# nmichlo/mtg-vision

Hardware: AMD Instinct MI355X
Metric: cards/sec end-to-end (detect+embed+top-1 over 100k bank), 640x640 (higher is better)
Workload: dtype f32 (products as 3 x f16 MFMA on hi/lo-split operands, f32 accumulate)

## Files before the change

### mtg-vision_amd/csrc/gemm_sp.hip

```cpp
#include "gemm_sp.h"

#include <stdlib.h>
#include <map>
#include <mutex>
#include <vector>

#include "gemm_sp_kernel.h"

namespace mtgv {

__global__ __launch_bounds__(256) void sp8_pack_rows_kernel(const float* __restrict__ in, sp_h8* __restrict__ out,
                                                           float* __restrict__ wscale, long rows, int K) {
  const int lane = threadIdx.x & 63;
  const long row = (long)blockIdx.x * 4 + (threadIdx.x >> 6);
  if (row >= rows) return;
  const float* x = in + row * K;
  float mx = 0.f;
  for (int k = lane; k < K; k += 64) mx = fmaxf(mx, fabsf(x[k]));
#pragma unroll
  for (int m = 32; m > 0; m >>= 1) mx = fmaxf(mx, __shfl_xor(mx, m));
  int e = 0;
  if (mx > 0.f && mx < INFINITY) {
    int ex;
    (void)frexpf(mx, &ex);
// ... 114 lines not shown
void gemm_sp_launch_cfg2(const SpDev& g, int amode, hipStream_t s);
void gemm_sp_launch_cfg3(const SpDev& g, int amode, hipStream_t s);
void gemm_sp_launch_cfg4(const SpDev& g, int amode, hipStream_t s);
void gemm_sp_launch_cfg5(const SpDev& g, int amode, hipStream_t s);
void gemm_sp_launch_cfg6(const SpDev& g, int amode, hipStream_t s);

namespace {
struct SpCfg {
  int wm, wn, tm, tn;
  double eff;
  int ks = 2;
  int bm() const { return 32 * tm * wm; }
  int bn() const { return 32 * tn * wn; }
  int rb() const { return 64 * ks; }
  int kps() const { return 16 * ks; }
};
const SpCfg kCfg[] = {
    {2, 2, 2, 2, 0.93},
    {2, 2, 2, 3, 1.00},
    {4, 1, 1, 3, 0.88},
    {4, 1, 1, 2, 0.80},
    {4, 1, 1, 1, 0.62},
    {4, 2, 1, 3, 0.00},
    {4, 1, 1, 1, 0.00, 1},
};
constexpr int kNumCfg = sizeof(kCfg) / sizeof(kCfg[0]);
}

bool window_conv_on() {
  static const bool on = [] { const char* e = getenv("MTGV_SP_WINDOW"); return e == nullptr || atoi(e) != 0; }();
  return on;
}

static size_t window_bytes(const SpCfg& k, int Wd) {
  const int rpp = 1024 / k.rb();
  return (size_t)((k.bm() + 2 * Wd + 2 + rpp - 1) / rpp * rpp) * k.rb();
}

bool window_conv_fits(const GemmArgs& a, const SpPlan& pl) {
  const SpCfg& k = kCfg[pl.cfg];
  if (!(window_conv_on() && a.KH == 3 && a.KW == 3 && a.stride == 1 && a.pad == 1 && a.stride_w <= 0 && a.Cin % k.kps() == 0 &&
        a.OH == a.H && a.OW == a.Wd))
    return false;
  return window_bytes(k, a.Wd) + (size_t)2 * k.bn() * k.rb() <= 80 * 1024;
}

bool gemm_sp_active() { return gemm_precision() == GEMM_PREC_F16X3; }

bool gemm_sp_takes_sp8(const float* W, int M, int N, int K, int lda, int c_off) {
  if (!gemm_sp_active()) return false;
  if (K % 8 != 0 || N % 4 != 0 || lda % 8 != 0 || c_off % 8 != 0 || M <= 0) return false;
  return sp8_lookup(W, K, nullptr, nullptr);
}

static int chain_cfg(const GemmArgs& a) {
  if (a.W2 == nullptr || a.Out2 == nullptr || !is_conv(a)) return -1;
  if (!(gemm_sp_active() && a.a_fmt == 1 && a.act == ACT_SILU && a.res == nullptr && a.grn_part == nullptr && a.topk == 0 && a.batch == 1 &&
        a.os == 1 && a.os_nq == 0 && a.OH2 == a.OH && a.OW2 == a.OW && a.a_scale == nullptr && a.ln_w == nullptr))
    return -1;
  if (!(a.N == 32 || a.N == 64 || a.N == 96) || a.N2 <= 0 || a.N2 % 32 != 0 || a.N2 > a.N) return -1;
  if (a.K % 8 != 0 || a.c_total % 8 != 0 || a.c_off % 8 != 0 || a.ldo2 % 4 != 0 || a.o_off2 % 4 != 0 || ((uintptr_t)a.Out2 & 15) != 0) return -1;
  if (a.out_fmt2 == 1 && (a.ldo2 % 8 != 0 || a.o_off2 % 8 != 0)) return -1;
  if (a.stride_w > 0 || a.Cin % 8 != 0) return -1;
  if (!sp8_lookup(a.W, a.K, nullptr, nullptr) || !sp8_lookup(a.W2, a.N, nullptr, nullptr)) return -1;
  return a.N == 32 ? 4 : (a.N == 64 ? 3 : 2);
}
bool gemm_sp_chain_ok(const GemmArgs& a) { return chain_cfg(a) >= 0; }

SpPlan gemm_sp_plan(const GemmArgs& a) {
  SpPlan pl;
  if (a.W2 != nullptr) {
    const int c = chain_cfg(a);
    MTGV_CHECK(c >= 0, ERR_INVALID, "gemm: this launch cannot chain its second layer (M=%d N=%d K=%d N2=%d): ask gemm_sp_chain_ok first", a.M,
               a.N, a.K, a.N2);
    const SpCfg& k = kCfg[c];
    pl.cfg = c, pl.bm = k.bm(), pl.bn = k.bn(), pl.unit_rows = 32 * k.tm;
    pl.tiles_m = ceil_div(a.M, k.bm()), pl.tiles_n = 1;
    return pl;
// ... 61 lines not shown
  if (best == 1 && !conv && sp8_in && a.grn_part != nullptr && a.topk == 0 && a.K >= 256 && a.M >= 12288) best = 5;
  const SpCfg& k = kCfg[best];
  pl.cfg = best;
  pl.bm = k.bm(), pl.bn = k.bn();
  pl.unit_rows = 32 * k.tm;
  pl.tiles_m = ceil_div(a.M, k.bm());
  pl.tiles_n = ceil_div(a.N, k.bn());
  return pl;
}

namespace {
struct StampRec { int M, N, K, cfg, amode, act, tiles; long* buf; };
std::vector<StampRec> g_stamps;
bool stamps_on() {
  static const bool on = [] { const char* e = getenv("MTGV_SP_STAMPS"); return e != nullptr && atoi(e) != 0; }();
  return on;
}
}

bool gemm_sp_topk_layout(const GemmArgs& a, int* slots, int* cols) {
  const SpPlan pl = gemm_sp_plan(a);
  if (pl.cfg < 0) return false;
  const SpCfg& k = kCfg[pl.cfg];
  *slots = pl.tiles_n * k.wn;
  *cols = 32 * k.tn;
  return true;
}

double gemm_sp_fill_bytes(const GemmArgs& a, const SpPlan& pl) {
  const SpCfg& k = kCfg[pl.cfg];
  const double tiles = (double)pl.tiles_m * pl.tiles_n;
  const double b_tile = (double)k.bn() * a.K * 4.0;
  double a_tile = (double)k.bm() * a.K * 4.0;
  if (a.a_fmt == 1 && is_conv(a) && window_conv_fits(a, pl)) a_tile = (double)window_bytes(k, a.Wd) * (a.Cin / k.kps());
  if (a.a_scale != nullptr) a_tile += (double)(a.K / 32) * 1024.0;
  return tiles * (a_tile + b_tile);
}

void gemm_sp_stamps_dump(const char* path) {
  if (g_stamps.empty()) return;
  HIP_OK(hipDeviceSynchronize());
  FILE* f = fopen(path, "wb");
  MTGV_CHECK(f != nullptr, ERR_RUNTIME, "cannot open %s", path);
  std::vector<long> host;
  for (const StampRec& r : g_stamps) {
    const int hdr[8] = {r.M, r.N, r.K, r.cfg, r.amode, r.act, r.tiles, 0};
    fwrite(hdr, sizeof(int), 8, f);
    host.resize((size_t)r.tiles * 8);
    HIP_OK(hipMemcpy(host.data(), r.buf, host.size() * sizeof(long), hipMemcpyDeviceToHost));
    fwrite(host.data(), sizeof(long), host.size(), f);
    HIP_OK(hipFree(r.buf));
  }
  fclose(f);
  g_stamps.clear();
}

int gemm_sp_topk_hi16_range_cols() { return 32 * kCfg[1].tn; }
int gemm_sp_topk_hi16_slots(int N) { return ceil_div(N, kCfg[1].bn()) * kCfg[1].wn; }

void gemm_sp_topk_hi16_launch(const void* q_hi, const void* bank_hi, const float* wscale, int b, int N, int K, int kp, float* cand_s,
                              int* cand_i, int* slots, hipStream_t s) {
  const SpCfg& k1 = kCfg[1];
  MTGV_CHECK(b >= 128 && N >= k1.bn() && K % 64 == 0 && kp >= 1 && kp <= 32 * k1.tn, ERR_INVALID, "topk_hi16: b=%d N=%d K=%d kp=%d", b, N, K, kp);
  MTGV_CHECK(((uintptr_t)q_hi & 15) == 0 && ((uintptr_t)bank_hi & 15) == 0, ERR_INVALID, "topk_hi16: operands must be 16-byte aligned");
  SpDev g;
  g.A = reinterpret_cast<const char*>(q_hi);
  g.a_rowb = (long)K * 2;
// ... 36 lines not shown
  g.d_hw = make_fastdiv((uint32_t)g.hw);
  g.a_scale = a.a_scale;
  g.a_mul = a.a_fmt == 1 ? 1.0f : a.a_mul;
  g.a_unmul = a.a_fmt == 1 ? 1.0f : a.a_unmul;
  g.zero = sp_zero_page();
  {
    const double lim = 4294967296.0 - 65536.0;
    g.off32 = ((double)a.M * g.a_rowb + (double)g.a_offb < lim && (double)a.N * a.K * 4.0 < lim) ? 1 : 0;
  }
  g.tiles_m = pl.tiles_m, g.tiles_n = pl.tiles_n;
  g.cand_s = a.cand_s, g.cand_i = a.cand_i, g.topk = a.topk;
  g.act = a.act;
  g.H = a.H, g.Wd = a.Wd, g.Cin = a.Cin, g.KW = a.KW, g.stride = a.stride, g.pad = a.pad, g.OH = a.OH, g.OW = a.OW;
  g.d_ohw = make_fastdiv((uint32_t)(a.OH * a.OW));
  g.d_ow = make_fastdiv((uint32_t)a.OW);
  g.d_cin = make_fastdiv((uint32_t)(a.Cin > 0 ? a.Cin : 1));
  g.d_kw = make_fastdiv((uint32_t)a.KW);
  g.remap = is_remap(a);
  g.os = a.os, g.oy = a.oy, g.ox = a.ox, g.OH2 = a.OH2, g.OW2 = a.OW2;
  if (a.W2 != nullptr) {
    const char* w28 = nullptr;
    const float* w2s = nullptr;
    MTGV_CHECK(sp8_lookup(a.W2, a.N, &w28, &w2s), ERR_RUNTIME, "gemm_sp: second-layer weights lost their SP8 copy");
    g.W2 = w28, g.wscale2 = w2s, g.bias2 = a.bias2, g.Out2 = a.Out2, g.ldo2 = a.ldo2, g.o_off2 = a.o_off2, g.out_fmt2 = a.out_fmt2;
    g.act2 = a.act2, g.N2 = a.N2;
  }
  g.nq = a.os_nq;
  g.d_nq = make_fastdiv((uint32_t)(a.os_nq > 0 ? a.os_nq : 1)), g.d_os = make_fastdiv((uint32_t)(a.os > 0 ? a.os : 1));
  if (a.os_nq > 0)
    MTGV_CHECK(g.remap && a.os_nq % 8 == 0 && a.N == a.os * a.os * a.os_nq && a.oy == 0 && a.ox == 0 && a.res == nullptr &&
                   a.grn_part == nullptr,
               ERR_INVALID, "gemm_sp: os_nq=%d does not describe a %dx%d scatter of N=%d columns", a.os_nq, a.os, a.os, a.N);
  int amode = a.a_fmt == 1 ? (is_conv(a) ? 2 : 0) : 1;
  if (amode == 2 && window_conv_fits(a, pl)) amode = 5;
  if (amode == 1 && g.a_mul == 1.0f && ((uintptr_t)g.A & 15) == 0) {
    if (g.a_scale == nullptr) amode = 4;
    else if (((uintptr_t)g.a_scale & 15) == 0 && (kCfg[pl.cfg].bm() - 1) / g.hw + 2 <= 8) amode = 3;
  }
  if (stamps_on() && gemm_profile_enabled()) {
    const int tiles = pl.tiles_m * pl.tiles_n;
    long* buf = nullptr;
    HIP_OK(hipMalloc(&buf, (size_t)tiles * 8 * sizeof(long)));
    HIP_OK(hipMemsetAsync(buf, 0, (size_t)tiles * 8 * sizeof(long), s));
    g.stamps = buf;
    g_stamps.push_back({a.M, a.N, a.K, pl.cfg, amode, a.act, tiles, buf});
  }
  switch (pl.cfg) {
    case 0: gemm_sp_launch_cfg0(g, amode, s); break;
    case 1: gemm_sp_launch_cfg1(g, amode, s); break;
    case 2: gemm_sp_launch_cfg2(g, amode, s); break;
    case 3: gemm_sp_launch_cfg3(g, amode, s); break;
    case 4: gemm_sp_launch_cfg4(g, amode, s); break;
    case 5: gemm_sp_launch_cfg5(g, amode, s); break;
    case 6: gemm_sp_launch_cfg6(g, amode, s); break;
    default: MTGV_CHECK(false, ERR_INVALID, "gemm_sp: bad cfg %d", pl.cfg);
  }
  HIP_OK(hipGetLastError());
}

}
```

### mtg-vision_amd/csrc/gemm_sp_inst.h

```cpp
#pragma once
#include "gemm_sp_kernel.h"

namespace mtgv {

namespace {
#ifndef SP_KS_VALUE
#define SP_KS_VALUE 2
#endif
constexpr int SP_KS = SP_KS_VALUE;
#ifndef SP_NST
#define SP_NST 2
#endif

template <int AMODE, int ACT, int EPI, int NST = SP_NST>
void sp_launch_nst(const SpDev& g, hipStream_t s) {
  constexpr int BM = 32 * SP_TM * SP_WM, BN = 32 * SP_TN * SP_WN;
  constexpr size_t ring = (size_t)NST * ((AMODE == 5 ? BN : BM + BN) * 64 * SP_KS + (AMODE == 3 ? 1024 : 0));
  size_t lds = ring;
  constexpr size_t chain_lds = (size_t)SP_WM * SP_WN * 4096 * (1 + SP_TN) + (size_t)SP_TN * 96 * 128;
  if (AMODE == 5) {
    constexpr int RB = 64 * SP_KS, RPP = 1024 / RB;
    const size_t win = (size_t)((BM + 2 * g.Wd + 2 + RPP - 1) / RPP * RPP) * RB;
    const size_t stage = (size_t)SP_WM * SP_WN * 32 * 128 * SP_TN;
    lds = win + ring > stage ? win + ring : stage;
  }
  if (EPI == 32 && lds < chain_lds) lds = chain_lds;
  static bool attr_done_dev[MTGV_MAX_DEVICES] = {};
  bool& attr_done = attr_done_dev[current_device()];
  auto kern = gemm_sp_kernel<SP_WM, SP_WN, SP_TM, SP_TN, SP_KS, NST, AMODE, ACT, EPI>;
  if (!attr_done) {
    HIP_OK(hipFuncSetAttribute((const void*)kern, hipFuncAttributeMaxDynamicSharedMemorySize, (AMODE == 5 || EPI == 32) ? 160 * 1024 : (int)lds));
    attr_done = true;
  }
  hipLaunchKernelGGL(kern, dim3((unsigned)(g.tiles_m * g.tiles_n)), dim3(64 * SP_WM * SP_WN), lds, s, g);
}

template <int AMODE, int ACT, int EPI>
void sp_launch_one(const SpDev& g, hipStream_t s) {
  if constexpr (AMODE == 5 && SP_NST == 2) {
    constexpr int BM = 32 * SP_TM * SP_WM, BN = 32 * SP_TN * SP_WN, RB = 64 * SP_KS, RPP = 1024 / RB;
    const size_t win = (size_t)((BM + 2 * g.Wd + 2 + RPP - 1) / RPP * RPP) * RB;
    if ((long)g.tiles_m * g.tiles_n <= 512 && win + (size_t)4 * BN * RB <= 80 * 1024) {
      sp_launch_nst<AMODE, ACT, EPI, 4>(g, s);
      return;
    }
  }
  sp_launch_nst<AMODE, ACT, EPI, SP_NST>(g, s);
}

int sp_epi_of(const SpDev& g) {
  if (g.W2 != nullptr) return 32;
  if (g.remap || g.N % 4 != 0) return -1;
  return (g.out_fmt == 1 ? 1 : 0) | (g.res != nullptr ? (g.res_fmt == 1 ? 4 : 2) : 0) | (g.grn_part != nullptr ? 8 : 0);
}

template <int AMODE, int ACT>
void sp_pick(const SpDev& g, int epi, hipStream_t s) {
  MTGV_CHECK(epi != 32, ERR_RUNTIME, "gemm_sp: no chained-1x1 instance for A mode %d in configuration %d", AMODE, SP_CFG_ID);
  sp_launch_one<AMODE, ACT, -1>(g, s);
}
template <int AMODE, int ACT, int E0, int... ES>
void sp_pick(const SpDev& g, int epi, hipStream_t s) {
  if (epi == E0) sp_launch_one<AMODE, ACT, E0>(g, s);
  else sp_pick<AMODE, ACT, ES...>(g, epi, s);
}
}

#define SP_CAT2(a, b) a##b
#define SP_CAT(a, b) SP_CAT2(a, b)

void SP_CAT(gemm_sp_launch_cfg, SP_CFG_ID)(const SpDev& g, int amode, hipStream_t s) {
  if (g.topk > 0) {
#if SP_CFG_ID == 1
    MTGV_CHECK((amode == 4 || amode == 6) && g.act == ACT_NONE, ERR_INVALID, "gemm_sp: top-k needs aligned f32 queries");
// ... 73 lines not shown
```

### mtg-vision_amd/csrc/gemm_sp_kernel.h

```cpp
#pragma once
#include <type_traits>

#include "act.h"
#include "gemm_f32.h"
#include "sp8.h"

namespace mtgv {

typedef float spf16 __attribute__((ext_vector_type(16)));

__device__ __forceinline__ spf16 sp_mfma(sp_h8 b, sp_h8 a, spf16 c) {
  return __builtin_amdgcn_mfma_f32_32x32x16_f16(b, a, c, 0, 0, 0);
}

struct SpDev {
  float* cand_s = nullptr;
  int* cand_i = nullptr;
  int topk = 0;
  long* stamps = nullptr;
  const char* A = nullptr;
  long a_rowb = 0;
  long a_offb = 0;
  const char* W = nullptr;
  const float* wscale = nullptr;
  const float* bias = nullptr;
  const void* res = nullptr;
  long ldr = 0;
  int res_fmt = 0;
  float* Out = nullptr;
  long ldo = 0;
  int o_off = 0;
  int out_fmt = 0;
  int M = 0, N = 0, K = 0;
  float* grn_part = nullptr;
  int hw = 1, segmax = 0;
  FastDiv d_hw;
  const float* a_scale = nullptr;
  float a_mul = 1.0f, a_unmul = 1.0f;
  const char* zero = nullptr;
  int off32 = 0;
  int tiles_m = 0, tiles_n = 0;
  int act = 0;
  int H = 1, Wd = 1, Cin = 0, KW = 1, stride = 1, pad = 0, OH = 1, OW = 1;
  FastDiv d_ohw, d_ow, d_cin, d_kw;
  int remap = 0, os = 1, oy = 0, ox = 0, OH2 = 1, OW2 = 1;
  int nq = 0;
  FastDiv d_nq, d_os;
  const char* W2 = nullptr;
  const float* wscale2 = nullptr;
  const float* bias2 = nullptr;
  float* Out2 = nullptr;
  long ldo2 = 0;
  int o_off2 = 0, out_fmt2 = 0, act2 = 0, N2 = 0;
};

typedef const __attribute__((address_space(1))) void* sp_gptr;
typedef __attribute__((address_space(3))) void* sp_lptr;

template <int WM, int WN, int TM, int TN, int KS, int NST, int AMODE, int ACT, int EPI>
__global__ __launch_bounds__(64 * WM * WN, (WM * WN == 8 ? 4 : 2)) void gemm_sp_kernel(const SpDev g) {
#pragma clang fp contract(off)
  constexpr int NW = WM * WN, NT = 64 * NW, BM = 32 * TM * WM, BN = 32 * TN * WN;
  constexpr bool GEN = EPI < 0;
  static_assert(TM <= 2, "the epilogue names its slabs");
  static_assert(NST >= 2 && NST <= 4 && (AMODE != 1 || NST == 2), "ring depth; the register A path is two-deep");
  constexpr int RB = 64 * KS, RPP = 1024 / RB, SPR = RB / 16;
  constexpr bool AWIN = AMODE == 5;
  constexpr bool ADMA = AMODE != 1 && !AWIN;
  constexpr bool AF32 = AMODE == 3 || AMODE == 4;
  constexpr bool HI16 = AMODE == 6;
  constexpr int EB = HI16 ? 2 : 4;
  static_assert(!HI16 || (KS == 2 && EPI == 16), "fp16 rows: 128-byte stage rows, top-k epilogue");
  constexpr int SA = AWIN ? 0 : BM * RB, SB = BN * RB, SSC = AMODE == 3 ? 1024 : 0, STG = SA + SB + SSC;
  static_assert(AMODE != 3 || KS == 2, "the scale image is one DMA piece: 8 images x 32 k");
  constexpr int PA = ADMA ? BM / RPP : 0, PB = BN / RPP, NP = PA + PB;
  constexpr int PPW = (NP + NW - 1) / NW;
  constexpr int CPS = BM * 2 * KS;
  constexpr int CPT = AMODE == 1 ? CPS / NT : 1;
  static_assert(AMODE != 1 || CPS % NT == 0, "A chunks must divide over the threads");
  extern __shared__ __attribute__((aligned(1024))) char smem[];

  const int tid = threadIdx.x, lane = tid & 63;
  const int wave = __builtin_amdgcn_readfirstlane(tid >> 6);
  const int wm = wave / WN, wn = wave % WN;
  const int r = lane & 31, h = lane >> 5;

  const long st0 = g.stamps != nullptr ? (long)__builtin_amdgcn_s_memtime() : 0;
  const long rt0 = g.stamps != nullptr ? (long)__builtin_amdgcn_s_memrealtime() : 0;
  long st1 = 0;
  int L;
  {
    const int nwg = gridDim.x, b = blockIdx.x;
    const int q = nwg >> 3, rr = nwg & 7, x = b & 7;
    L = (x < rr ? x * (q + 1) : rr * (q + 1) + (x - rr) * q) + (b >> 3);
  }
  const int tile_n = L % g.tiles_n, tile_m = L / g.tiles_n;
  const int m0 = tile_m * BM, n0 = tile_n * BN;
  const long wrowb = (long)g.K * EB;
  const int kchunks = g.K >> 3;
  constexpr int KPS = 16 * KS * (4 / EB);
  const int nk = (g.K + KPS - 1) / KPS;
  const bool ktail = (g.K % KPS) != 0;

  const char* src[PPW];
  bool tailz[PPW];
  int cslot[PPW], cih0[PPW], ciw0[PPW];
  const char* csrc[PPW];
  const bool conv_fast = AMODE == 2 && g.Cin % (16 * KS) == 0;
  uint32_t off32[PPW];
  const bool sfast = g.off32 != 0 && !ktail;
#pragma unroll
  for (int u = 0; u < PPW; ++u) {
    const int p = wave + NW * u;
    const bool isA = p < PA;
    const int pp = isA ? p : p - PA;
    const int row = pp * RPP + lane / SPR;
    const int sw = KS == 2 ? (row >> 1) & 7 : (row >> 2) & 3;
    const int slot = (lane % SPR) ^ sw;
    cslot[u] = slot, cih0[u] = 0, ciw0[u] = 0, csrc[u] = nullptr;
    {
      const int mm = m0 + row < g.M ? m0 + row : g.M - 1, nn = n0 + row < g.N ? n0 + row : g.N - 1;
      off32[u] = isA ? (uint32_t)mm * (uint32_t)g.a_rowb + (uint32_t)(slot * 16) : (uint32_t)nn * (uint32_t)wrowb + (uint32_t)(slot * 16);
    }
    if (isA) {
      int m = m0 + row;
      m = m < g.M ? m : g.M - 1;
      if constexpr (AMODE == 2) {
        const uint32_t img = fdiv((uint32_t)m, g.d_ohw);
        const uint32_t rem = (uint32_t)m - img * (uint32_t)(g.OH * g.OW);
        const uint32_t oh = fdiv(rem, g.d_ow);
        const uint32_t ow = rem - oh * (uint32_t)g.OW;
        cih0[u] = (int)oh * g.stride - g.pad;
        ciw0[u] = (int)ow * g.stride - g.pad;
        csrc[u] = g.A + (((long)img * g.H + cih0[u]) * g.Wd + ciw0[u]) * g.a_rowb + g.a_offb + slot * 16;
        src[u] = g.A + (long)img * g.H * g.Wd * g.a_rowb + g.a_offb + (slot & 1) * 16;
      } else {
        src[u] = g.A + (long)m * g.a_rowb + g.a_offb + slot * 16;
      }
    } else {
      int n = n0 + row;
      n = n < g.N ? n : g.N - 1;
      src[u] = g.W + (long)n * wrowb + slot * 16;
    }
    tailz[u] = ktail && ((nk - 1) * 2 * KS + (slot >> 1)) >= kchunks;
  }
  const int img0 = AMODE == 3 ? (int)fdiv((uint32_t)m0, g.d_hw) : 0;
  const char* sc_src = nullptr;
  bool sc_tailz = false;
  if constexpr (AMODE == 3) {
    const int img_last = (int)fdiv((uint32_t)(g.M - 1), g.d_hw);
    const int im = img0 + (lane >> 3) < img_last ? img0 + (lane >> 3) : img_last;
    sc_src = reinterpret_cast<const char*>(g.a_scale + (long)im * g.K) + (lane & 7) * 16;
    sc_tailz = ktail && ((nk - 1) * 2 * KS + ((lane & 7) >> 1)) >= kchunks;
  }
  const int win_px = AWIN ? ((BM + 2 * g.Wd + 2 + RPP - 1) / RPP * RPP) : 0;
  char* const ring = smem + (AWIN ? win_px * RB : 0);
  auto issue_piece = [&](int u, int t, int buf) {
    const int p = wave + NW * u;
    const char* s;
    if (AMODE == 2 && p < PA && conv_fast) {
      const uint32_t k0 = (uint32_t)t * (16u * KS);
      const uint32_t tap = fdiv(k0, g.d_cin);
      const uint32_t kh = fdiv(tap, g.d_kw);
      const uint32_t kw = tap - kh * (uint32_t)g.KW;
      const long tap_off = ((long)kh * g.Wd + kw) * g.a_rowb + (long)(k0 - tap * (uint32_t)g.Cin) * 4;
      const bool ok = (unsigned)(cih0[u] + (int)kh) < (unsigned)g.H && (unsigned)(ciw0[u] + (int)kw) < (unsigned)g.Wd;
      s = ok ? csrc[u] + tap_off : g.zero;
    } else if (AMODE == 2 && p < PA) {
      const int kc = t * 2 * KS + (cslot[u] >> 1);
      const uint32_t k = (uint32_t)(kc < kchunks ? kc : 0) * 8u;
      const uint32_t tap = fdiv(k, g.d_cin);
      const uint32_t c = k - tap * (uint32_t)g.Cin;
      const uint32_t kh = fdiv(tap, g.d_kw);
      const uint32_t kw = tap - kh * (uint32_t)g.KW;
      const int ih = cih0[u] + (int)kh, iw = ciw0[u] + (int)kw;
      const bool ok = kc < kchunks && ih >= 0 && ih < g.H && iw >= 0 && iw < g.Wd;
      s = ok ? src[u] + ((long)ih * g.Wd + iw) * g.a_rowb + c * 4 : g.zero;
    } else {
      s = src[u] + (long)t * RB;
      if (t == nk - 1 && tailz[u]) s = g.zero;
    }
    __builtin_amdgcn_global_load_lds((sp_gptr)s, (sp_lptr)(ring + buf * STG + (SA - PA * 1024) + p * 1024), 16, 0, 0);
  };
  auto issue = [&](int t, int buf) {
    if (sfast) {
      const char* const abase = g.A + g.a_offb + (long)t * RB;
      const char* const wbase = g.W + (long)t * RB;
#pragma unroll
// ... 46 lines not shown
        ra[v][0] = ra[v][1] = z;
        rs[v][0] = rs[v][1] = z;
        if (ok) {
          const sp_f4* p = reinterpret_cast<const sp_f4*>(a_ptr[v] + (long)t * RB);
          ra[v][0] = p[0], ra[v][1] = p[1];
          if (g.a_scale != nullptr) {
            const sp_f4* q = reinterpret_cast<const sp_f4*>(s_ptr[v] + t * 16 * KS);
            rs[v][0] = q[0], rs[v][1] = q[1];
          }
        }
      }
    }
  };
  auto storeA = [&](int buf) {
    if constexpr (AMODE == 1) {
#pragma unroll
      for (int v = 0; v < CPT; ++v) {
        sp_h8 hi, lo;
        if (g.a_scale != nullptr)
          sp8_split8(ra[v][0] * rs[v][0] * g.a_mul, ra[v][1] * rs[v][1] * g.a_mul, hi, lo);
        else
          sp8_split8(ra[v][0] * g.a_mul, ra[v][1] * g.a_mul, hi, lo);
        char* const d = ring + buf * STG;
        *reinterpret_cast<sp_h8*>(d + a_lds[v]) = hi;
        *reinterpret_cast<sp_h8*>(d + (a_lds[v] ^ 16u)) = lo;
      }
    }
  };

  auto issue_window = [&](int cc) {
    if constexpr (AWIN) {
      for (int pw = wave; pw < win_px / RPP; pw += NW) {
        const int w = pw * RPP + lane / SPR;
        const long gp = (long)m0 - g.Wd - 1 + w;
        const int slot = (lane % SPR) ^ (KS == 2 ? (w >> 1) & 7 : (w >> 2) & 3);
        const char* sp = (gp >= 0 && gp < (long)g.M) ? g.A + gp * g.a_rowb + g.a_offb + cc * RB + slot * 16 : g.zero;
        __builtin_amdgcn_global_load_lds((sp_gptr)sp, (sp_lptr)(smem + pw * 1024), 16, 0, 0);
      }
    }
  };
  if constexpr (AWIN) {
    const int ncc0 = g.Cin / (16 * KS);
#pragma unroll
    for (int s0 = 0; s0 < NST - 1; ++s0)
      if (s0 < 9 * ncc0) issue((s0 % 9) * ncc0 + s0 / 9, s0);
    issue_window(0);
  } else {
#pragma unroll
    for (int s0 = 0; s0 < NST - 1; ++s0)
      if (s0 < nk) issue(s0, s0);
    loadA(0);
  }
  int wy[TM], wx[TM];
#pragma unroll
  for (int i = 0; i < TM; ++i) {
    wy[i] = wx[i] = 0;
    if constexpr (AWIN) {
      int m = m0 + wm * TM * 32 + i * 32 + r;
      m = m < g.M ? m : g.M - 1;
      const uint32_t img = fdiv((uint32_t)m, g.d_ohw);
      const uint32_t rem = (uint32_t)m - img * (uint32_t)(g.OH * g.OW);
      wy[i] = (int)fdiv(rem, g.d_ow);
      wx[i] = (int)(rem - (uint32_t)wy[i] * (uint32_t)g.OW);
    }
  }

  spf16 acc[TM][TN];
#pragma unroll
  for (int i = 0; i < TM; ++i)
#pragma unroll
    for (int j = 0; j < TN; ++j)
#pragma unroll
      for (int q = 0; q < 16; ++q) acc[i][j][q] = 0.f;

  const int swr = KS == 2 ? (r >> 1) & 7 : (r >> 2) & 3;
  unsigned a_off[TM], b_off[TN];
#pragma unroll
  for (int i = 0; i < TM; ++i) a_off[i] = (unsigned)((wm * TM * 32 + i * 32 + r) * RB);
#pragma unroll
  for (int j = 0; j < TN; ++j) b_off[j] = (unsigned)(SA + (wn * TN * 32 + j * 32 + r) * RB);
  unsigned sc_off[TM];
#pragma unroll
  for (int i = 0; i < TM; ++i) {
    sc_off[i] = 0;
    if constexpr (AMODE == 3) {
      int m = m0 + wm * TM * 32 + i * 32 + r;
      m = m < g.M ? m : g.M - 1;
      sc_off[i] = (unsigned)(SA + SB + ((int)fdiv((uint32_t)m, g.d_hw) - img0) * 128 + h * 32);
    }
  }

  const int nw0 = n0 + wn * TN * 32;
  const int mw0 = m0 + wm * TM * 32;
  const int slot = lane & 7, lrow = lane >> 3;
  sp_f4 wsc[TN], bsv[TN];
  bool col_ok[TN];
// ... 34 lines not shown
      asm volatile("s_waitcnt vmcnt(%0) lgkmcnt(0)" ::"n"(PPW * AHEAD) : "memory");
    } else if (my_pieces == PPW + 1) {
      asm volatile("s_waitcnt vmcnt(%0) lgkmcnt(0)" ::"n"((PPW + 1) * AHEAD) : "memory");
    } else {
      asm volatile("s_waitcnt vmcnt(%0) lgkmcnt(0)" ::"n"((PPW > 1 ? PPW - 1 : 0) * AHEAD) : "memory");
    }
  };

  if constexpr (AWIN) {
    const int ncc = g.Cin / (16 * KS);
    const int ntau = 9 * ncc;
    const char* const win = smem;
    int buf = 0, nbuf = NST - 1;
    int tau = 0;
    for (int cc = 0; cc < ncc; ++cc) {
      if (cc > 0) {
        __builtin_amdgcn_s_barrier();
        issue_window(cc);
      }
      for (int tap = 0; tap < 9; ++tap, ++tau) {
        if (tap == 0) asm volatile("s_waitcnt vmcnt(0) lgkmcnt(0)" ::: "memory");
        else wait_stage(tau + NST - 1 > ntau);
        __builtin_amdgcn_s_barrier();
        if (g.stamps != nullptr && cc == 0 && tap == 0) st1 = (long)__builtin_amdgcn_s_memtime();
        {
          const int ta = tau + NST - 1;
          if (ta < ntau) {
            const int ca = ta / 9;
            issue((ta - ca * 9) * ncc + ca, nbuf);
          }
        }
        if (wave_active) {
          const int dy = tap / 3 - 1, dx = tap - (tap / 3) * 3 - 1;
          const int shift = g.Wd + 1 + dy * g.Wd + dx;
          const char* const sb = ring + buf * STG;
          unsigned w_off[TM], w_sw[TM];
          bool w_ok[TM];
#pragma unroll
          for (int i = 0; i < TM; ++i) {
            const int w = wm * TM * 32 + i * 32 + r + shift;
            w_off[i] = (unsigned)w * (unsigned)RB;
            w_sw[i] = KS == 2 ? (unsigned)(w >> 1) & 7u : (unsigned)(w >> 2) & 3u;
            w_ok[i] = (unsigned)(wy[i] + dy) < (unsigned)g.H && (unsigned)(wx[i] + dx) < (unsigned)g.Wd;
          }
#pragma unroll
          for (int ks = 0; ks < KS; ++ks) {
            const unsigned shi = (unsigned)(((ks * 4 + h * 2 + 0) ^ swr) << 4);
            const unsigned slo = (unsigned)(((ks * 4 + h * 2 + 1) ^ swr) << 4);
            sp_h8 ah[TM], al[TM], bh[TN], bl[TN];
            const sp_h8 z8 = {0, 0, 0, 0, 0, 0, 0, 0};
#pragma unroll
            for (int i = 0; i < TM; ++i) {
              const sp_h8 vh = *reinterpret_cast<const sp_h8*>(win + w_off[i] + (((ks * 4 + h * 2 + 0) ^ w_sw[i]) << 4));
              const sp_h8 vl = *reinterpret_cast<const sp_h8*>(win + w_off[i] + (((ks * 4 + h * 2 + 1) ^ w_sw[i]) << 4));
              ah[i] = w_ok[i] ? vh : z8;
              al[i] = w_ok[i] ? vl : z8;
            }
#pragma unroll
            for (int j = 0; j < TN; ++j) {
              bh[j] = *reinterpret_cast<const sp_h8*>(sb + b_off[j] + shi);
              bl[j] = *reinterpret_cast<const sp_h8*>(sb + b_off[j] + slo);
            }
#pragma unroll
            for (int j = 0; j < TN; ++j)
#pragma unroll
              for (int i = 0; i < TM; ++i) {
                acc[i][j] = sp_mfma(bl[j], ah[i], acc[i][j]);
                acc[i][j] = sp_mfma(bh[j], al[i], acc[i][j]);
                acc[i][j] = sp_mfma(bh[j], ah[i], acc[i][j]);
              }
          }
        }
        buf = buf + 1 == NST ? 0 : buf + 1;
        nbuf = nbuf + 1 == NST ? 0 : nbuf + 1;
      }
// ... 114 lines not shown
          for (int j = 0; j < TN; ++j) {
            bh[j] = *reinterpret_cast<const sp_h8*>(sb + b_off[j] + shi);
            bl[j] = *reinterpret_cast<const sp_h8*>(sb + b_off[j] + slo);
          }
  #pragma unroll
          for (int j = 0; j < TN; ++j)
  #pragma unroll
            for (int i = 0; i < TM; ++i) acc[i][j] = sp_mfma(bl[j], ah[i], acc[i][j]);
  #pragma unroll
          for (int j = 0; j < TN; ++j)
  #pragma unroll
            for (int i = 0; i < TM; ++i) acc[i][j] = sp_mfma(bh[j], al[i], acc[i][j]);
  #pragma unroll
          for (int j = 0; j < TN; ++j)
  #pragma unroll
            for (int i = 0; i < TM; ++i) acc[i][j] = sp_mfma(bh[j], ah[i], acc[i][j]);
        }
      }
      if (AMODE == 1 && t + 1 < nk) storeA(buf ^ 1);
      buf = buf + 1 == NST ? 0 : buf + 1;
      nbuf = nbuf + 1 == NST ? 0 : nbuf + 1;
    }
  }

  auto activate = [&](float x) -> float {
    if constexpr (ACT == ACT_NONE) return x;
    else if constexpr (ACT == ACT_GELU) return act_gelu(x);
    else if constexpr (ACT == ACT_MISH) return act_mish(x);
    else if constexpr (ACT == ACT_SILU) return act_silu(x);
    else return apply_act(x, g.act);
  };
  __builtin_amdgcn_s_barrier();
  const long st2 = g.stamps != nullptr ? (long)__builtin_amdgcn_s_memtime() : 0;

  if constexpr (EPI == 32) {
    static_assert(EPI != 32 || (WN == 1 && TM == 1 && KS == 2 && !HI16), "chained 1x1: one wave holds whole rows");
    constexpr int CB = 32 * 128;
    char* const stg1 = smem + wave * CB;
    char* const a2 = smem + NW * CB + wave * (TN * CB);
    char* const w2 = smem + NW * CB * (1 + TN);
    const int n2g = g.N2 >> 3;
    for (int p = wave; p < TN * n2g; p += NW) {
      const int s = p / n2g, rg = p - s * n2g;
      const int row = rg * 8 + (lane >> 3);
      const int slot_s = (lane & 7) ^ ((row >> 1) & 7);
      const char* const sp = g.W2 + (long)row * ((long)g.N * 4) + s * 128 + slot_s * 16;
      __builtin_amdgcn_global_load_lds((sp_gptr)sp, (sp_lptr)(w2 + s * (g.N2 * 128) + rg * 1024), 16, 0, 0);
    }
    const int slot = lane & 7, lrow = lane >> 3;
    const int mw0 = m0 + wm * 32;
    if (wave_active) {
#pragma unroll
      for (int j = 0; j < TN; ++j) {
        const int n = n0 + j * 32 + slot * 4;
        const sp_f4 w1 = *reinterpret_cast<const sp_f4*>(g.wscale + n);
        const sp_f4 b1 = g.bias != nullptr ? *reinterpret_cast<const sp_f4*>(g.bias + n) : sp_f4{0.f, 0.f, 0.f, 0.f};
#pragma unroll
        for (int gq = 0; gq < 4; ++gq)
          *reinterpret_cast<sp_f4*>(stg1 + r * 128 + (((gq * 2 + h) ^ (r & 7)) << 4)) =
              sp_f4{acc[0][j][4 * gq], acc[0][j][4 * gq + 1], acc[0][j][4 * gq + 2], acc[0][j][4 * gq + 3]};
#pragma unroll
        for (int it = 0; it < 4; ++it) {
          const int row = it * 8 + lrow;
          const sp_f4 raw = *reinterpret_cast<const sp_f4*>(stg1 + row * 128 + ((slot ^ lrow) << 4));
          sp_f4 v;
#pragma unroll
// ... 27 lines not shown
          bh[j] = *reinterpret_cast<const sp_h8*>(w2 + s * (g.N2 * 128) + rowb * 128 + shi);
          bl[j] = *reinterpret_cast<const sp_h8*>(w2 + s * (g.N2 * 128) + rowb * 128 + slo);
        }
#pragma unroll
        for (int j = 0; j < TN; ++j) acc2[j] = __builtin_amdgcn_mfma_f32_32x32x16_f16(bl[j], ah, acc2[j], 0, 0, 0);
#pragma unroll
        for (int j = 0; j < TN; ++j) acc2[j] = __builtin_amdgcn_mfma_f32_32x32x16_f16(bh[j], al, acc2[j], 0, 0, 0);
#pragma unroll
        for (int j = 0; j < TN; ++j) acc2[j] = __builtin_amdgcn_mfma_f32_32x32x16_f16(bh[j], ah, acc2[j], 0, 0, 0);
      }
    }
#pragma unroll
    for (int j = 0; j < TN; ++j) {
      if (j >= tn2) break;
      const int n = j * 32 + slot * 4;
      const sp_f4 w1 = *reinterpret_cast<const sp_f4*>(g.wscale2 + n);
      const sp_f4 b1 = g.bias2 != nullptr ? *reinterpret_cast<const sp_f4*>(g.bias2 + n) : sp_f4{0.f, 0.f, 0.f, 0.f};
#pragma unroll
      for (int gq = 0; gq < 4; ++gq)
        *reinterpret_cast<sp_f4*>(stg1 + r * 128 + (((gq * 2 + h) ^ (r & 7)) << 4)) =
            sp_f4{acc2[j][4 * gq], acc2[j][4 * gq + 1], acc2[j][4 * gq + 2], acc2[j][4 * gq + 3]};
#pragma unroll
      for (int it = 0; it < 4; ++it) {
        const int m = mw0 + it * 8 + lrow;
        const sp_f4 raw = *reinterpret_cast<const sp_f4*>(stg1 + (it * 8 + lrow) * 128 + ((slot ^ lrow) << 4));
        sp_f4 v;
#pragma unroll
        for (int e = 0; e < 4; ++e) {
          const float t = __builtin_fmaf(raw[e], w1[e], b1[e]);
          v[e] = g.act2 == ACT_SILU ? act_silu(t) : (g.act2 == ACT_NONE ? t : apply_act(t, g.act2));
        }
        sp_f4 piece = v;
        if (g.out_fmt2 == 1) piece = __builtin_bit_cast(sp_f4, sp8_piece_from_quad(v, slot));
        if (m < g.M) *reinterpret_cast<sp_f4*>(g.Out2 + (long)m * g.ldo2 + g.o_off2 + n) = piece;
      }
    }
    return;
  }
  if (!wave_active) return;

  if constexpr (EPI == 16) {
    const int ncol0 = n0 + wn * TN * 32;
#pragma unroll
    for (int j = 0; j < TN; ++j)
#pragma unroll
      for (int gq = 0; gq < 4; ++gq) {
        const int n = ncol0 + j * 32 + gq * 8 + 4 * h;
#pragma unroll
        for (int e = 0; e < 4; ++e) {
          const bool nok = n + e < g.N;
          const float ws = (g.wscale != nullptr && nok) ? g.wscale[n + e] * g.a_unmul : g.a_unmul;
#pragma unroll
          for (int i = 0; i < TM; ++i) acc[i][j][4 * gq + e] = nok ? acc[i][j][4 * gq + e] * ws : -INFINITY;
        }
      }
    const long slots = (long)g.tiles_n * WN;
#pragma unroll
    for (int i = 0; i < TM; ++i) {
      const int m = m0 + wm * TM * 32 + i * 32 + r;
      for (int kk = 0; kk < g.topk; ++kk) {
        float bs = -INFINITY;
        int bi = 0x7fffffff;
#pragma unroll
        for (int j = 0; j < TN; ++j)
#pragma unroll
          for (int q = 0; q < 16; ++q) {
            const float v = acc[i][j][q];
// ... 7 lines not shown
          const long o = ((long)m * slots + (long)tile_n * WN + wn) * g.topk + kk;
          g.cand_s[o] = bs;
          g.cand_i[o] = (bs == -INFINITY) ? -1 : bi;
        }
#pragma unroll
        for (int j = 0; j < TN; ++j)
#pragma unroll
          for (int q = 0; q < 16; ++q)
            if (ncol0 + j * 32 + (q >> 2) * 8 + 4 * h + (q & 3) == bi) acc[i][j][q] = -INFINITY;
      }
    }
    return;
  }

  constexpr int SROW = 128 * TN;
  constexpr int WREG = 32 * SROW;
  constexpr int ER = (!AWIN && NW * WREG > NST * STG) ? 2 : 1;
  static_assert(AWIN || (NW / ER) * WREG <= NST * STG, "the store staging area must fit into the ring");
  char* const stg = smem + (ER == 1 ? wave : wave % (NW / ER)) * WREG;
  if constexpr (ER == 2) {
    if (wave >= NW / 2) __builtin_amdgcn_s_barrier();
  }
  constexpr int NIT = 4;

  const bool out_sp8 = GEN ? g.out_fmt == 1 : (EPI & 1) != 0;
  const bool res_f32 = GEN ? (g.res != nullptr && g.res_fmt == 0) : (EPI & 2) != 0;
  const bool res_sp8 = GEN ? (g.res != nullptr && g.res_fmt == 1) : (EPI & 4) != 0;
  const bool has_res = res_f32 || res_sp8;
  const bool remap = GEN ? g.remap : false;
  const bool grn = GEN ? g.grn_part != nullptr : (EPI & 8) != 0;
  const int img_first = grn ? (int)fdiv((uint32_t)mw0, g.d_hw) : 0;
  const long unit = (long)tile_m * WM + wm;
  const int ncol0 = nw0 + slot * 4;
  const long o_lane = (long)(mw0 + lrow) * g.ldo + g.o_off + ncol0;
  const long r_lane = (long)(mw0 + lrow) * g.ldr + ncol0;
  const char* const stg_rd = stg + lrow * SROW + ((slot ^ lrow) << 4);

  auto load_res = [&](int i, int j, sp_f4 (&rr)[NIT]) {
#pragma unroll
    for (int it = 0; it < NIT; ++it) {
      rr[it] = sp_f4{0.f, 0.f, 0.f, 0.f};
      const long e = r_lane + (long)(i * 32 + it * 8) * g.ldr + j * 32;
      if (col_ok[j] && mw0 + i * 32 + it * 8 + lrow < g.M) {
        if (res_f32) {
          rr[it] = *reinterpret_cast<const sp_f4*>(reinterpret_cast<const float*>(g.res) + e);
        } else if (res_sp8) {
          typedef float f2 __attribute__((ext_vector_type(2)));
          const char* const c = reinterpret_cast<const char*>(g.res) + (e - 4 * (slot & 1)) * 4 + 8 * (slot & 1);
          const f2 hi = *reinterpret_cast<const f2*>(c), lo = *reinterpret_cast<const f2*>(c + 16);
          rr[it] = sp_f4{hi[0], hi[1], lo[0], lo[1]};
        }
      }
    }
  };

  sp_f4 run[TN];
#pragma unroll
  for (int j = 0; j < TN; ++j) run[j] = sp_f4{0.f, 0.f, 0.f, 0.f};
  int run_seg = 0;
  auto flush = [&]() {
#pragma unroll
    for (int j = 0; j < TN; ++j) {
      sp_f4 t = run[j];
#pragma unroll
      for (int e = 0; e < 4; ++e)
#pragma unroll
        for (int mask = 8; mask < 64; mask <<= 1) t[e] += __shfl_xor(t[e], mask);
      if (lane < 8 && col_ok[j])
        *reinterpret_cast<sp_f4*>(g.grn_part + (unit * g.segmax + run_seg) * g.N + ncol0 + j * 32) = t;
      run[j] = sp_f4{0.f, 0.f, 0.f, 0.f};
    }
  };

  sp_f4 rcur[NIT], rnext[NIT];
  if (has_res) load_res(0, 0, rcur);
// ... 18 lines not shown
      constexpr int NB = TM * TN;
      const int bnext = i * TN + j + 1;
      if (has_res && bnext < NB) load_res(bnext / TN, bnext % TN, rnext);
#pragma unroll
      for (int it = 0; it < NIT; ++it) {
        const int m = ms0 + it * 8 + lrow;
        const bool ok = FAST || (col_ok[j] && m < g.M);
        const sp_f4 raw = *reinterpret_cast<const sp_f4*>(stg_rd + j * 128 + it * 8 * SROW);
        sp_f4 v;
#pragma unroll
        for (int e = 0; e < 4; ++e)
          v[e] = activate(__builtin_fmaf(raw[e], wsc[j][e], bsv[j][e]));
        if (grn) {
          if (single) {
            if (ok) {
#pragma unroll
              for (int e = 0; e < 4; ++e) run[j][e] = __builtin_fmaf(v[e], v[e], run[j][e]);
            }
          } else {
            *reinterpret_cast<sp_f4*>(stg + (it * 8 + lrow) * SROW + (((j * 8 + slot) ^ lrow) << 4)) = v;
          }
        }
        if (res_f32) {
          v = v + rcur[it];
        } else if (res_sp8) {
          typedef _Float16 h4 __attribute__((ext_vector_type(4)));
          typedef float f2 __attribute__((ext_vector_type(2)));
          const h4 rh = __builtin_bit_cast(h4, f2{rcur[it][0], rcur[it][1]}), rl = __builtin_bit_cast(h4, f2{rcur[it][2], rcur[it][3]});
          v = v + (__builtin_convertvector(rh, sp_f4) + __builtin_convertvector(rl, sp_f4));
        }
        sp_f4 piece = v;
        if (out_sp8) piece = __builtin_bit_cast(sp_f4, sp8_piece_from_quad(v, slot));
        if (ok) {
          const long drow = i * 32 + it * 8;
          if (remap) {
            const uint32_t img = fdiv((uint32_t)m, g.d_ohw);
            const uint32_t rem = (uint32_t)m - img * (uint32_t)(g.OH * g.OW);
            const uint32_t oh = fdiv(rem, g.d_ow);
            const uint32_t ow = rem - oh * (uint32_t)g.OW;
            uint32_t oy = (uint32_t)g.oy, ox = (uint32_t)g.ox, cn = (uint32_t)(ncol0 + j * 32);
            if (g.nq > 0) {
              const uint32_t q = fdiv(cn, g.d_nq);
              cn -= q * (uint32_t)g.nq;
              oy = fdiv(q, g.d_os);
              ox = q - oy * (uint32_t)g.os;
            }
            const long orow = ((long)img * g.OH2 + oh * g.os + oy) * g.OW2 + ow * g.os + ox;
            *reinterpret_cast<sp_f4*>(g.Out + orow * g.ldo + g.o_off + cn) = piece;
          } else if (!GEN || ncol0 + j * 32 + 4 <= g.N) {
            *reinterpret_cast<sp_f4*>(g.Out + o_lane + drow * g.ldo + j * 32) = piece;
          } else {
#pragma unroll
            for (int e = 0; e < 4; ++e)
              if (ncol0 + j * 32 + e < g.N) g.Out[o_lane + drow * g.ldo + j * 32 + e] = piece[e];
          }
        }
      }
      if (has_res && bnext < NB) {
#pragma unroll
        for (int it = 0; it < NIT; ++it) rcur[it] = rnext[it];
      }
    }
    if (!FAST && grn && !single) {
      for (int sgm = seg_lo; sgm <= seg_hi; ++sgm) {
        if (sgm != run_seg) {
          flush();
          run_seg = sgm;
// ... 63 lines not shown
```

Measured before the change: 32560.

## Use 2-D spatial tiles for windowed 3x3 conv A-operand staging

```diff
diff --git a/mtg-vision_amd/csrc/gemm_sp.hip b/mtg-vision_amd/csrc/gemm_sp.hip
--- a/mtg-vision_amd/csrc/gemm_sp.hip
+++ b/mtg-vision_amd/csrc/gemm_sp.hip
@@ -170,18 +170,26 @@
   return on;
 }
 
-static size_t window_bytes(const SpCfg& k, int Wd) {
-  const int rpp = 1024 / k.rb();
-  return (size_t)((k.bm() + 2 * Wd + 2 + rpp - 1) / rpp * rpp) * k.rb();
-}
-
-bool window_conv_fits(const GemmArgs& a, const SpPlan& pl) {
+enum { SP_WIN_NONE = 0, SP_WIN_LINEAR = 1, SP_WIN_2D = 2 };
+
+bool window2d_on() {
+  static const bool on = [] { const char* e = getenv("MTGV_SP_WINDOW2D"); return e == nullptr || atoi(e) != 0; }();
+  return on;
+}
+
+static size_t window_bytes(const SpCfg& k, int Wd, bool win2d) { return (size_t)sp_window_pixels(k.bm(), Wd, k.ks, win2d) * k.rb(); }
+
+int window_conv_form(const GemmArgs& a, const SpPlan& pl) {
   const SpCfg& k = kCfg[pl.cfg];
-  if (!(window_conv_on() && a.KH == 3 && a.KW == 3 && a.stride == 1 && a.pad == 1 && a.stride_w <= 0 && a.Cin % k.kps() == 0 &&
-        a.OH == a.H && a.OW == a.Wd))
-    return false;
-  return window_bytes(k, a.Wd) + (size_t)2 * k.bn() * k.rb() <= 80 * 1024;
-}
+  if (!(window_conv_on() && a.a_fmt == 1 && a.KH == 3 && a.KW == 3 && a.stride == 1 && a.pad == 1 && a.stride_w <= 0 &&
+        a.Cin % k.kps() == 0 && a.OH == a.H && a.OW == a.Wd))
+    return SP_WIN_NONE;
+  if (window_bytes(k, a.Wd, false) + (size_t)2 * k.bn() * k.rb() > 80 * 1024) return SP_WIN_NONE;
+  const bool tiles2d = k.wm == 4 && k.tm == 1 && a.Wd % SP_W2D_TW == 0 && a.H % SP_W2D_TH == 0 && a.M % (a.H * a.Wd) == 0;
+  if (window2d_on() && tiles2d && !is_remap(a) && a.grn_part == nullptr && a.topk == 0) return SP_WIN_2D;
+  return SP_WIN_LINEAR;
+}
+bool window_conv_fits(const GemmArgs& a, const SpPlan& pl) { return window_conv_form(a, pl) != SP_WIN_NONE; }
 
 bool gemm_sp_active() { return gemm_precision() == GEMM_PREC_F16X3; }
 
@@ -309,7 +317,10 @@
   const double tiles = (double)pl.tiles_m * pl.tiles_n;
   const double b_tile = (double)k.bn() * a.K * 4.0;
   double a_tile = (double)k.bm() * a.K * 4.0;
-  if (a.a_fmt == 1 && is_conv(a) && window_conv_fits(a, pl)) a_tile = (double)window_bytes(k, a.Wd) * (a.Cin / k.kps());
+  if (a.a_fmt == 1 && is_conv(a)) {
+    const int form = window_conv_form(a, pl);
+    if (form != SP_WIN_NONE) a_tile = (double)window_bytes(k, a.Wd, form == SP_WIN_2D) * (a.Cin / k.kps());
+  }
   if (a.a_scale != nullptr) a_tile += (double)(a.K / 32) * 1024.0;
   return tiles * (a_tile + b_tile);
 }
@@ -412,7 +423,15 @@
                    a.grn_part == nullptr,
                ERR_INVALID, "gemm_sp: os_nq=%d does not describe a %dx%d scatter of N=%d columns", a.os_nq, a.os, a.os, a.N);
   int amode = a.a_fmt == 1 ? (is_conv(a) ? 2 : 0) : 1;
-  if (amode == 2 && window_conv_fits(a, pl)) amode = 5;
+  if (amode == 2) {
+    const int form = window_conv_form(a, pl);
+    if (form != SP_WIN_NONE) amode = 5;
+    if (form == SP_WIN_2D) {
+      g.win2d = 1;
+      g.tpx = a.Wd / SP_W2D_TW, g.tpi = (a.H / SP_W2D_TH) * g.tpx;
+      g.d_tpx = make_fastdiv((uint32_t)g.tpx), g.d_tpi = make_fastdiv((uint32_t)g.tpi);
+    }
+  }
   if (amode == 1 && g.a_mul == 1.0f && ((uintptr_t)g.A & 15) == 0) {
     if (g.a_scale == nullptr) amode = 4;
     else if (((uintptr_t)g.a_scale & 15) == 0 && (kCfg[pl.cfg].bm() - 1) / g.hw + 2 <= 8) amode = 3;
diff --git a/mtg-vision_amd/csrc/gemm_sp_inst.h b/mtg-vision_amd/csrc/gemm_sp_inst.h
--- a/mtg-vision_amd/csrc/gemm_sp_inst.h
+++ b/mtg-vision_amd/csrc/gemm_sp_inst.h
@@ -19,8 +19,7 @@
   size_t lds = ring;
   constexpr size_t chain_lds = (size_t)SP_WM * SP_WN * 4096 * (1 + SP_TN) + (size_t)SP_TN * 96 * 128;
   if (AMODE == 5) {
-    constexpr int RB = 64 * SP_KS, RPP = 1024 / RB;
-    const size_t win = (size_t)((BM + 2 * g.Wd + 2 + RPP - 1) / RPP * RPP) * RB;
+    const size_t win = (size_t)sp_window_pixels(BM, g.Wd, SP_KS, g.win2d != 0) * (64 * SP_KS);
     const size_t stage = (size_t)SP_WM * SP_WN * 32 * 128 * SP_TN;
     lds = win + ring > stage ? win + ring : stage;
   }
@@ -38,8 +37,8 @@
 template <int AMODE, int ACT, int EPI>
 void sp_launch_one(const SpDev& g, hipStream_t s) {
   if constexpr (AMODE == 5 && SP_NST == 2) {
-    constexpr int BM = 32 * SP_TM * SP_WM, BN = 32 * SP_TN * SP_WN, RB = 64 * SP_KS, RPP = 1024 / RB;
-    const size_t win = (size_t)((BM + 2 * g.Wd + 2 + RPP - 1) / RPP * RPP) * RB;
+    constexpr int BM = 32 * SP_TM * SP_WM, BN = 32 * SP_TN * SP_WN, RB = 64 * SP_KS;
+    const size_t win = (size_t)sp_window_pixels(BM, g.Wd, SP_KS, g.win2d != 0) * RB;
     if ((long)g.tiles_m * g.tiles_n <= 512 && win + (size_t)4 * BN * RB <= 80 * 1024) {
       sp_launch_nst<AMODE, ACT, EPI, 4>(g, s);
       return;
diff --git a/mtg-vision_amd/csrc/gemm_sp_kernel.h b/mtg-vision_amd/csrc/gemm_sp_kernel.h
--- a/mtg-vision_amd/csrc/gemm_sp_kernel.h
+++ b/mtg-vision_amd/csrc/gemm_sp_kernel.h
@@ -52,7 +52,45 @@
   float* Out2 = nullptr;
   long ldo2 = 0;
   int o_off2 = 0, out_fmt2 = 0, act2 = 0, N2 = 0;
+  int win2d = 0, tpi = 1, tpx = 1;
+  FastDiv d_tpi, d_tpx;
 };
+
+constexpr int SP_W2D_TW = 16, SP_W2D_TH = 8;
+#ifndef MTGV_SP_W2D_PITCH
+#define MTGV_SP_W2D_PITCH 24
+#endif
+__host__ __device__ constexpr int sp_win2d_pitch(int ks) { return ks == 2 ? MTGV_SP_W2D_PITCH : 20; }
+__host__ __device__ constexpr int sp_win_key(int ks, int c) { return ks == 2 ? (c >> 1) & 7 : (c >> 2) & 3; }
+__host__ __device__ constexpr int sp_win2d_pixel(int l, int tap, int P) { return (l / SP_W2D_TW + tap / 3) * P + l % SP_W2D_TW + tap % 3; }
+__host__ __device__ constexpr int sp_win2d_col(int l, int tap) { return l % SP_W2D_TW + tap % 3; }
+__host__ __device__ constexpr int sp_window_pixels(int bm, int Wd, int ks, bool win2d) {
+  const int rpp = 16 / ks;
+  const int px = win2d ? (SP_W2D_TH + 2) * sp_win2d_pitch(ks) : bm + 2 * Wd + 2;
+  return (px + rpp - 1) / rpp * rpp;
+}
+constexpr bool sp_win2d_conflict_free(int ks) {
+  const int P = sp_win2d_pitch(ks), rb = 64 * ks, spr = rb / 16;
+  if (P < SP_W2D_TW + 2 || P % (ks == 2 ? 2 : 4) != 0) return false;
+  const int grp[2][16] = {{0, 1, 2, 3, 12, 13, 14, 15, 20, 21, 22, 23, 24, 25, 26, 27},
+                          {4, 5, 6, 7, 8, 9, 10, 11, 16, 17, 18, 19, 28, 29, 30, 31}};
+  for (int wm = 0; wm < 4; ++wm)
+    for (int gi = 0; gi < 4; ++gi)
+      for (int tap = 0; tap < 9; ++tap)
+        for (int s = 0; s < 2 * ks; ++s) {
+          unsigned seen = 0;
+          for (int q = 0; q < 16; ++q) {
+            const int lane = grp[gi & 1][q] + 32 * (gi >> 1), l = wm * 32 + (lane & 31), h = lane >> 5;
+            const int slot = ((s >> 1) * 4 + h * 2 + (s & 1)) ^ sp_win_key(ks, sp_win2d_col(l, tap));
+            if (slot >= spr) return false;
+            const int bank16 = ((sp_win2d_pixel(l, tap, P) * rb + slot * 16) / 16) % 16;
+            if (seen & (1u << bank16)) return false;
+            seen |= 1u << bank16;
+          }
+        }
+  return true;
+}
+static_assert(sp_win2d_conflict_free(1) && sp_win2d_conflict_free(2), "2-D window: a fragment read would hit a bank group twice");
 
 typedef const __attribute__((address_space(1))) void* sp_gptr;
 typedef __attribute__((address_space(3))) void* sp_lptr;
@@ -96,6 +134,20 @@
   }
   const int tile_n = L % g.tiles_n, tile_m = L / g.tiles_n;
   const int m0 = tile_m * BM, n0 = tile_n * BN;
+  constexpr bool W2D_OK = AWIN && WM == 4 && TM == 1;
+  constexpr int WP = sp_win2d_pitch(KS);
+  const bool w2d = W2D_OK && g.win2d != 0;
+  int wy0 = 0, wx0 = 0, mbase = m0;
+  if constexpr (W2D_OK) {
+    if (w2d) {
+      const uint32_t img = fdiv((uint32_t)tile_m, g.d_tpi);
+      const uint32_t rem = (uint32_t)tile_m - img * (uint32_t)g.tpi;
+      const uint32_t ty = fdiv(rem, g.d_tpx);
+      wy0 = (int)ty * SP_W2D_TH;
+      wx0 = (int)(rem - ty * (uint32_t)g.tpx) * SP_W2D_TW;
+      mbase = ((int)img * g.H + wy0) * g.Wd + wx0;
+    }
+  }
   const long wrowb = (long)g.K * EB;
   const int kchunks = g.K >> 3;
   constexpr int KPS = 16 * KS * (4 / EB);
@@ -153,7 +205,7 @@
     sc_src = reinterpret_cast<const char*>(g.a_scale + (long)im * g.K) + (lane & 7) * 16;
     sc_tailz = ktail && ((nk - 1) * 2 * KS + ((lane & 7) >> 1)) >= kchunks;
   }
-  const int win_px = AWIN ? ((BM + 2 * g.Wd + 2 + RPP - 1) / RPP * RPP) : 0;
+  const int win_px = AWIN ? sp_window_pixels(BM, g.Wd, KS, w2d) : 0;
   char* const ring = smem + (AWIN ? win_px * RB : 0);
   auto issue_piece = [&](int u, int t, int buf) {
     const int p = wave + NW * u;
@@ -266,9 +318,20 @@
     if constexpr (AWIN) {
       for (int pw = wave; pw < win_px / RPP; pw += NW) {
         const int w = pw * RPP + lane / SPR;
-        const long gp = (long)m0 - g.Wd - 1 + w;
-        const int slot = (lane % SPR) ^ (KS == 2 ? (w >> 1) & 7 : (w >> 2) & 3);
-        const char* sp = (gp >= 0 && gp < (long)g.M) ? g.A + gp * g.a_rowb + g.a_offb + cc * RB + slot * 16 : g.zero;
+        long gp = (long)m0 - g.Wd - 1 + w;
+        bool ok = gp >= 0 && gp < (long)g.M;
+        int key = sp_win_key(KS, w);
+        if constexpr (W2D_OK) {
+          if (w2d) {
+            const int wr = w / WP, wc = w - wr * WP;
+            ok = wr < SP_W2D_TH + 2 && wc < SP_W2D_TW + 2 && (unsigned)(wy0 - 1 + wr) < (unsigned)g.H &&
+                 (unsigned)(wx0 - 1 + wc) < (unsigned)g.Wd;
+            gp = (long)mbase + (long)(wr - 1) * g.Wd + (wc - 1);
+            key = sp_win_key(KS, wc);
+          }
+        }
+        const int slot = (lane % SPR) ^ key;
+        const char* sp = ok ? g.A + gp * g.a_rowb + g.a_offb + cc * RB + slot * 16 : g.zero;
         __builtin_amdgcn_global_load_lds((sp_gptr)sp, (sp_lptr)(smem + pw * 1024), 16, 0, 0);
       }
     }
@@ -290,12 +353,17 @@
   for (int i = 0; i < TM; ++i) {
     wy[i] = wx[i] = 0;
     if constexpr (AWIN) {
-      int m = m0 + wm * TM * 32 + i * 32 + r;
-      m = m < g.M ? m : g.M - 1;
-      const uint32_t img = fdiv((uint32_t)m, g.d_ohw);
-      const uint32_t rem = (uint32_t)m - img * (uint32_t)(g.OH * g.OW);
-      wy[i] = (int)fdiv(rem, g.d_ow);
-      wx[i] = (int)(rem - (uint32_t)wy[i] * (uint32_t)g.OW);
+      if (w2d) {
+        const int l = wm * TM * 32 + i * 32 + r;
+        wy[i] = wy0 + l / SP_W2D_TW, wx[i] = wx0 + l % SP_W2D_TW;
+      } else {
+        int m = m0 + wm * TM * 32 + i * 32 + r;
+        m = m < g.M ? m : g.M - 1;
+        const uint32_t img = fdiv((uint32_t)m, g.d_ohw);
+        const uint32_t rem = (uint32_t)m - img * (uint32_t)(g.OH * g.OW);
+        wy[i] = (int)fdiv(rem, g.d_ow);
+        wx[i] = (int)(rem - (uint32_t)wy[i] * (uint32_t)g.OW);
+      }
     }
   }
 
@@ -396,15 +464,19 @@
         }
         if (wave_active) {
           const int dy = tap / 3 - 1, dx = tap - (tap / 3) * 3 - 1;
-          const int shift = g.Wd + 1 + dy * g.Wd + dx;
+          const int pitch = w2d ? WP : g.Wd;
+          const int shift = pitch + 1 + dy * pitch + dx;
+          const int kshift = w2d ? 1 + dx : shift;
+          const int rowskip = w2d ? WP - SP_W2D_TW : 0, kmask = w2d ? SP_W2D_TW - 1 : -1;
           const char* const sb = ring + buf * STG;
           unsigned w_off[TM], w_sw[TM];
           bool w_ok[TM];
 #pragma unroll
           for (int i = 0; i < TM; ++i) {
-            const int w = wm * TM * 32 + i * 32 + r + shift;
+            const int l = wm * TM * 32 + i * 32 + r;
+            const int w = l + (l >> 4) * rowskip + shift;
             w_off[i] = (unsigned)w * (unsigned)RB;
-            w_sw[i] = KS == 2 ? (unsigned)(w >> 1) & 7u : (unsigned)(w >> 2) & 3u;
+            w_sw[i] = (unsigned)sp_win_key(KS, (l & kmask) + kshift);
             w_ok[i] = (unsigned)(wy[i] + dy) < (unsigned)g.H && (unsigned)(wx[i] + dx) < (unsigned)g.Wd;
           }
 #pragma unroll
@@ -585,6 +657,8 @@
   };
   __builtin_amdgcn_s_barrier();
   const long st2 = g.stamps != nullptr ? (long)__builtin_amdgcn_s_memtime() : 0;
+  const int mrow0 = (W2D_OK && w2d) ? mbase + wm * (32 / SP_W2D_TW) * g.Wd : m0 + wm * TM * 32;
+  auto tile_drow = [&](int q) -> int { return (W2D_OK && w2d) ? (q / SP_W2D_TW) * g.Wd + q % SP_W2D_TW : q; };
 
   if constexpr (EPI == 32) {
     static_assert(EPI != 32 || (WN == 1 && TM == 1 && KS == 2 && !HI16), "chained 1x1: one wave holds whole rows");
@@ -678,7 +752,7 @@
         }
         sp_f4 piece = v;
         if (g.out_fmt2 == 1) piece = __builtin_bit_cast(sp_f4, sp8_piece_from_quad(v, slot));
-        if (m < g.M) *reinterpret_cast<sp_f4*>(g.Out2 + (long)m * g.ldo2 + g.o_off2 + n) = piece;
+        if (m < g.M) *reinterpret_cast<sp_f4*>(g.Out2 + (long)(mrow0 + tile_drow(it * 8) + lrow) * g.ldo2 + g.o_off2 + n) = piece;
       }
     }
     return;
@@ -752,15 +826,15 @@
   const int img_first = grn ? (int)fdiv((uint32_t)mw0, g.d_hw) : 0;
   const long unit = (long)tile_m * WM + wm;
   const int ncol0 = nw0 + slot * 4;
-  const long o_lane = (long)(mw0 + lrow) * g.ldo + g.o_off + ncol0;
-  const long r_lane = (long)(mw0 + lrow) * g.ldr + ncol0;
+  const long o_lane = (long)(mrow0 + lrow) * g.ldo + g.o_off + ncol0;
+  const long r_lane = (long)(mrow0 + lrow) * g.ldr + ncol0;
   const char* const stg_rd = stg + lrow * SROW + ((slot ^ lrow) << 4);
 
   auto load_res = [&](int i, int j, sp_f4 (&rr)[NIT]) {
 #pragma unroll
     for (int it = 0; it < NIT; ++it) {
       rr[it] = sp_f4{0.f, 0.f, 0.f, 0.f};
-      const long e = r_lane + (long)(i * 32 + it * 8) * g.ldr + j * 32;
+      const long e = r_lane + (long)tile_drow(i * 32 + it * 8) * g.ldr + j * 32;
       if (col_ok[j] && mw0 + i * 32 + it * 8 + lrow < g.M) {
         if (res_f32) {
           rr[it] = *reinterpret_cast<const sp_f4*>(reinterpret_cast<const float*>(g.res) + e);
@@ -845,7 +919,7 @@
         sp_f4 piece = v;
         if (out_sp8) piece = __builtin_bit_cast(sp_f4, sp8_piece_from_quad(v, slot));
         if (ok) {
-          const long drow = i * 32 + it * 8;
+          const long drow = tile_drow(i * 32 + it * 8);
           if (remap) {
             const uint32_t img = fdiv((uint32_t)m, g.d_ohw);
             const uint32_t rem = (uint32_t)m - img * (uint32_t)(g.OH * g.OW);
```

Result: no change. 32430 (-0.4%).
